# voxel-tracer/ag-pathtracer

Hardware: AMD Instinct MI355X
Metric: Mrays/sec (primary+secondary) at 1080p/64spp (higher is better)
Workload: dtype f32; 1 GPU; BASELINE configs[2]: Sponza-class closed atrium, 258672 tris / 37 primitives / 35 Disney materials, 1920x1080, 64 spp, PathTracer MaxDepth=5, NEE+MIS; triangles=258672, spp=64

## Files before the change

### ag-pathtracer_amd/csrc/agpt_api.hip

```cpp
#include <hip/hip_runtime.h>

#include <algorithm>
#include <cstdlib>
#include <cstring>
#include <memory>
#include <string>
#include <vector>

#include "agpt_adaptive.h"
#include "agpt_denoise.h"
#include "agpt_internal.h"
#include "agpt_kernels.h"
#include "agpt_motion.h"

namespace agpt {

static thread_local std::string g_error;

int fail(int code, const std::string& msg) {
    g_error = msg;
    return code;
}

int interleave_rows(int H, int block, int world, int rank) {
// ... 209 lines not shown
    if (!c || !dst || !src) return fail(AGPT_ERR_INVALID, "agpt_device_download: NULL argument");
    HIP_TRY(hipMemcpyAsync(dst, src, bytes, hipMemcpyDeviceToHost, c->stream));
    HIP_TRY(hipStreamSynchronize(c->stream));
    return AGPT_OK;
}
int agpt_device_upload(agpt_ctx* c, void* dst, const void* src, size_t bytes) {
    if (!c || !dst || !src) return fail(AGPT_ERR_INVALID, "agpt_device_upload: NULL argument");
    HIP_TRY(hipMemcpyAsync(dst, src, bytes, hipMemcpyHostToDevice, c->stream));
    HIP_TRY(hipStreamSynchronize(c->stream));
    return AGPT_OK;
}

#define X(T, name) +sizeof(T)
constexpr size_t AGPT_BYTES_PER_PATH = (0 AGPT_POOL_BUFFERS(X)) + 2 * AGPT_NQUEUES * sizeof(uint32_t);
#undef X
static_assert(AGPT_BYTES_PER_PATH == 240, "11 float4 arrays + 2 hit arrays (16 B) + 2 flag words + 6 queue words");
static size_t candidate_bytes_per_path(int n_prims) { return n_prims > 64 ? 4 + 8 * (size_t)((n_prims + 63) / 64) : 0; }
static int ensure_pool(agpt_ctx* c, size_t paths, int n_prims) {
    int rc;
    paths = std::max(paths, c->pool_paths);
    if (n_prims > 64) {
        if ((rc = c->cand_chunks.ensure(paths))) return rc;
        if ((rc = c->cand_mask.ensure(paths * (size_t)((n_prims + 63) / 64)))) return rc;
    }
#define X(T, name) \
    if ((rc = c->name.ensure(paths))) return rc;
    AGPT_POOL_BUFFERS(X)
#undef X
    for (int i = 0; i < 2; i++)
        for (int j = 0; j < AGPT_NQUEUES; j++)
            if ((rc = c->q[i][j].ensure(paths))) return rc;
// ... 100 lines not shown
            uint32_t* slot = c->host_pinned + (it & 1) * (AGPT_NQUEUES * AGPT_QSTRIDE);
            HIP_TRY(hipMemcpyAsync(slot, q[cur].counts, ((AGPT_NQUEUES - 1) * AGPT_QSTRIDE + 1) * sizeof(uint32_t), hipMemcpyDeviceToHost, main_stream));
            HIP_TRY(hipEventRecord(c->ev[2 + (it & 1)], main_stream));
            if (it > planned) {
                const uint32_t* seen = c->host_pinned + ((it - 1) & 1) * (AGPT_NQUEUES * AGPT_QSTRIDE);
                HIP_TRY(hipEventSynchronize(c->ev[2 + ((it - 1) & 1)]));
                if (seen[0] == 0 && seen[AGPT_QSTRIDE] == 0 && seen[2 * AGPT_QSTRIDE] == 0) break;
            }
            if (it > 4096) return fail(AGPT_ERR_LIMIT, "agpt: path did not terminate");
        }
        const int nxt = cur ^ 1;
        HIP_TRY(hipMemsetAsync(q[nxt].counts, 0, AGPT_NQUEUES * AGPT_QSTRIDE * sizeof(uint32_t), main_stream));
        HIP_TRY(hipMemsetAsync(c->work.p, 0, 4 * AGPT_FRONTIERS * AGPT_QSTRIDE * sizeof(uint32_t), main_stream));
        uint32_t* const heads[4] = {c->work.p, c->work.p + AGPT_FRONTIERS * AGPT_QSTRIDE, c->work.p + 2 * AGPT_FRONTIERS * AGPT_QSTRIDE,
                                    c->work.p + 3 * AGPT_FRONTIERS * AGPT_QSTRIDE};
        const TraceLaunch ext{main_stream, q[cur].ext, &QCOUNT(q[cur], 0), 0, heads[0], pb.ext_o, pb.ext_d, pb.hit, nullptr,
                              count, small_batch, recast, coherent && it == 0};
        const TraceLaunch mis{mis_stream, q[cur].mis, &QCOUNT(q[cur], 1), 0, heads[1], pb.mis_o, pb.mis_d,
                              run.mis_mode ? nullptr : pb.mis_hit, run.mis_mode ? pb.mis_ok : nullptr, count, small_batch, false, false};
        const TraceLaunch shadow{shadow_stream, q[cur].shadow, &QCOUNT(q[cur], 2), 0, heads[2], pb.sh_o, pb.sh_d, nullptr, pb.occluded,
                                 count, small_batch, false, false};
        auto trace_ext = [&]() { launch_trace_timed<0>(c, run.timing, 0, s->dev, ext); };
        auto trace_mis = [&]() {
            if (run.mis_mode) launch_trace_timed<2>(c, run.timing, 1, s->dev, mis);
            else launch_trace_timed<0>(c, run.timing, 1, s->dev, mis);
        };
        auto trace_shadow = [&]() { launch_trace_timed<1>(c, run.timing, 2, s->dev, shadow); };
        if (side) {
            HIP_TRY(hipEventRecord(c->aux_ev[0], main_stream));
            HIP_TRY(hipStreamWaitEvent(mis_stream, c->aux_ev[0], 0));
            HIP_TRY(hipStreamWaitEvent(shadow_stream, c->aux_ev[0], 0));
            trace_mis();
            HIP_TRY(hipEventRecord(c->aux_ev[1], mis_stream));
            trace_shadow();
            HIP_TRY(hipEventRecord(c->aux_ev[2], shadow_stream));
            trace_ext();
            HIP_TRY(hipStreamWaitEvent(main_stream, c->aux_ev[1], 0));
            HIP_TRY(hipStreamWaitEvent(main_stream, c->aux_ev[2], 0));
        } else {
            trace_ext();
            trace_mis();
            trace_shadow();
        }
        agpt::launch_shading(main_stream, run.shade, shade_grid, s->dev, rcn, pb, q[cur], q[nxt], c->counters.p, heads[3]);
        cur = nxt;
        run.iterations++;
        run.launches += 3;
    }
    return AGPT_OK;
}

static void read_counters(const DevCounters& d, agpt_stats* st) {
    st->closest_rays = d.closest_rays;
    st->anyhit_rays = d.anyhit_rays;
    st->interior_visits = d.interior;
    st->root_tests = d.roots;
    st->tri_tests = d.tris;
    st->shaded_vertices = d.shaded;
    st->outliers = d.outliers;
// ... 419 lines not shown
```

### ag-pathtracer_amd/csrc/agpt_internal.h

```cpp
#pragma once

#include <hip/hip_runtime.h>

#include <string>
#include <utility>
#include <vector>

#include "../../include/agpt.h"
#include "agpt_host_scene.hpp"
#include "agpt_update.h"
#include "agpt_wavefront.h"

#ifndef AGPT_FAST_STACK
#define AGPT_FAST_STACK 23
#endif
#ifndef AGPT_FAST_BLOCKS_PER_CU
#define AGPT_FAST_BLOCKS_PER_CU 5
#endif
#define AGPT_REFILL 20
#define AGPT_REFILL_ANY 40

namespace agpt {
int fail(int code, const std::string& msg);
int interleave_rows(int H, int block, int world, int rank);
// ... 42 lines not shown
    }
    int in(const T* host, size_t count) {
        HIP_TRY(alloc(count));
        HIP_TRY(hipMemcpy(p, host, count * sizeof(T), hipMemcpyHostToDevice));
        return AGPT_OK;
    }
    int out(T* host, size_t count, const hipStream_t* st = nullptr) const {
        if (st) HIP_TRY(hipMemcpyAsync(host, p, count * sizeof(T), hipMemcpyDeviceToHost, *st));
        else HIP_TRY(hipMemcpy(host, p, count * sizeof(T), hipMemcpyDeviceToHost));
        return AGPT_OK;
    }
};

#define AGPT_POOL_BUFFERS(X)                                                                                                  \
    X(float4, ext_o) X(float4, ext_d) X(float4, sh_o) X(float4, sh_d) X(float4, mis_o) X(float4, mis_d) X(float4, beta4)      \
    X(float4, L4) X(float4, fac4) X(float4, c1) X(float4, c2) X(DevHit, hit) X(DevHit, mis_hit) X(uint32_t, occluded)          \
    X(uint32_t, mis_ok)

struct agpt_ctx {
    int device = 0;
    hipStream_t stream = nullptr;
    int num_cus = 256;
    hipEvent_t ev[4] = {nullptr, nullptr, nullptr, nullptr};
    hipStream_t aux_stream[2] = {nullptr, nullptr};
    hipEvent_t aux_ev[3] = {nullptr, nullptr, nullptr};
    int multi_stream = 0;
    size_t pool_paths = 0;
#define X(T, name) DevBuf<T> name;
    AGPT_POOL_BUFFERS(X)
#undef X
    DevBuf<uint32_t> q[2][AGPT_NQUEUES];
// ... 111 lines not shown
```

### ag-pathtracer_amd/csrc/agpt_kernels.h

```cpp
#pragma once

#include <type_traits>

#include "agpt_shade.h"
#include "agpt_trace.h"

#include "agpt_wavefront.h"

template <bool ANY, bool COUNT, int DEPTH>
__global__ void __launch_bounds__(AGPT_BLOCK)
k_trace(DevScene sc, const uint32_t* __restrict__ queue, const uint32_t* __restrict__ count_ptr, uint32_t count_imm,
        uint32_t* __restrict__ work_head, const float4* __restrict__ ray_o, const float4* __restrict__ ray_d,
        DevHit* __restrict__ hits, uint32_t* __restrict__ occluded, DevCounters* __restrict__ counters) {
    __shared__ uint32_t s_stack[DEPTH * AGPT_BLOCK];
    uint32_t* stack = s_stack + threadIdx.x;
    const int lane = threadIdx.x & 63;
    const uint32_t count = count_ptr ? *count_ptr : count_imm;
    TraceCounters cnt;
    cnt.interior = 0;
    cnt.tris = 0;
    cnt.roots = 0;
    cnt.last_mesh = 0;
    for (;;) {
        uint32_t base = 0;
// ... 307 lines not shown
    for (;;) {
        TCK(const unsigned long long tk_r0 = TCK_NOW();)
        pin_state();
        any_slow = uni(any_slow);
        if constexpr (MODE == 0 && !LIST) {
            if (__ballot(cur == CUR_RECAST) != 0 && cur == CUR_RECAST) {
                const v3 p = r.O + rayt * r.D;
                const v3 nO = p + AGPT_EPSILON * r.D;
                const v3 nD = normalize(r.D);
                const TraceRay nr = make_trace_ray(nO, nD, coords_ok);
                if (nr.fast) {
                    const float kind = ray_d[pid].w;
                    if (kind == 2.f) {
                        const int al = sc.prims[hid & 0x7FFFFFFFu].arealight;
                        const v3 Le = al >= 0 ? V3(sc.lights[al].L[0], sc.lights[al].L[1], sc.lights[al].L[2]) : V3s(0.f);
                        const float4 b4 = path_beta4[pid];
                        float4 l4 = path_L4[pid];
                        const v3 L = V3(l4.x, l4.y, l4.z) + V3(b4.x, b4.y, b4.z) * Le;
                        l4.x = L.x; l4.y = L.y; l4.z = L.z;
                        path_L4[pid] = l4;
                    }
                    float4 no4, nd4;
                    no4.x = nO.x; no4.y = nO.y; no4.z = nO.z; no4.w = AGPT_FLT_MAX;
                    nd4.x = nD.x; nd4.y = nD.y; nd4.z = nD.z; nd4.w = kind;
                    ray_o[pid] = no4;
                    ray_d[pid] = nd4;
                    atomicAdd(&counters->closest_rays, 1ull);
                    r = nr;
                    rayt = AGPT_FLT_MAX;
                    hid = AGPT_HIT_MISS;
                    hb1 = 0.f;
                    hb2 = 0.f;
                    sp = 0;
// ... 497 lines not shown
    float py = y + rng_float(rng);
    float s = px / rc.W, t = py / rc.H;
    v3 O, D;
    camera_sample_ray(sc.cam, s, t, rng, O, D);
    start_path(pb, q, i, total, O, D, AGPT_FLT_MAX, rng, rc.max_depth);
}

__global__ void __launch_bounds__(AGPT_BLOCK)
k_generate_li(const agpt_ray* __restrict__ rays, const uint32_t* __restrict__ rng_states, uint32_t n, PathBuffers pb, Queues q, int max_depth) {
    const uint32_t i = blockIdx.x * blockDim.x + threadIdx.x;
    if (i >= n) return;
    const agpt_ray r = rays[i];
    const v3 d = normalize(V3(r.d[0], r.d[1], r.d[2]));
    start_path(pb, q, i, n, V3(r.o[0], r.o[1], r.o[2]), d, r.tmax, rng_states[i], max_depth);
}

__global__ void k_resolve(const float4* __restrict__ accum, int n, int samples, uint32_t* __restrict__ out) {
    int i = blockIdx.x * blockDim.x + threadIdx.x;
    if (i >= n) return;
    out[i] = resolve_word(accum[i], (float)samples);
}
```

### ag-pathtracer_amd/csrc/agpt_shade_kernels.h

```cpp
#pragma once

#include "agpt_shade.h"
#include "agpt_trace.h"
#include "agpt_wavefront.h"

#define AGPT_SHADE_LEVEL_LIST(X) X(0, ) X(1, _textured) X(2, _mapped) X(3, _sampled) X(4, _normal)
#ifndef AGPT_SHADE_LEVEL
#define AGPT_SHADE_LEVEL 0
#endif
#if AGPT_SHADE_FAST
#define AGPT_SHADE_FAST_SUFFIX _fast
#else
#define AGPT_SHADE_FAST_SUFFIX
#endif
#define AGPT_SHADE_NTH_0(s0, ...) s0
#define AGPT_SHADE_NTH_1(s0, s1, ...) s1
#define AGPT_SHADE_NTH_2(s0, s1, s2, ...) s2
#define AGPT_SHADE_NTH_3(s0, s1, s2, s3, ...) s3
#define AGPT_SHADE_NTH_4(s0, s1, s2, s3, s4, ...) s4
#define AGPT_SHADE_SUFFIX_ARG(level, suffix) suffix,
#define AGPT_SHADE_CAT_(a, b, c) a##b##c
#define AGPT_SHADE_CAT(a, b, c) AGPT_SHADE_CAT_(a, b, c)
#define AGPT_SHADE_NTH(n, list) AGPT_SHADE_CAT(AGPT_SHADE_NTH_, n, )(list)
#define AGPT_SHADE_KNAME(n) AGPT_SHADE_CAT(n, AGPT_SHADE_NTH(AGPT_SHADE_LEVEL, AGPT_SHADE_LEVEL_LIST(AGPT_SHADE_SUFFIX_ARG)), AGPT_SHADE_FAST_SUFFIX)

#define SB_EXT 1u
#define SB_MIS 2u
#define SB_SHADOW 4u
#define SB_SHADED 32u
#define SB_MIS_ANSWERED 64u
#define SB_RAY_ANSWERED 128u

__device__ __forceinline__ v3 pending_light_sample(const DevScene& sc, const RenderConsts& rc, const PathBuffers& pb, uint32_t pid,
                                                   uint32_t flags, uint32_t was_occluded, uint32_t was_mis_ok, float4 c1_4, float4 c2_4,
                                                   float4 f4) {
    v3 Ld = V3s(0.f);
    if (flags & PF_PEND_C1) {
        if (!was_occluded) {
            Ld = Ld + V3(c1_4.x, c1_4.y, c1_4.z);
        }
    }
    if (flags & PF_PEND_C2) {
        uint32_t light = __float_as_uint(f4.w);
        bool add;
        if (rc.mis_mode) {
            add = was_mis_ok != 0;
        } else if (uint32_t hid = pb.mis_hit[pid].id; hid != AGPT_HIT_MISS) {
            int hp = (hid & AGPT_HIT_SPHERE) ? (int)(hid & 0x7FFFFFFFu)
                                             : (int)__float_as_uint(sc.tri_shade[4 * (size_t)hid + 3].w);
            add = sc.prims[hp].arealight == (int)light;
        } else {
            add = sc.lights[light].type != AGPT_LIGHT_AREA;
        }
        if (add) Ld = Ld + V3(c2_4.x, c2_4.y, c2_4.z);
    }
    return Ld;
}

#ifdef AGPT_SHADE_CLOCK
#define SCK_PARAMS , unsigned long long* sck_acc, unsigned long long& sck_last
#define SCK_ARGS , sck_acc, sck_last
#define SCK(k) do { asm volatile("s_waitcnt vmcnt(0) lgkmcnt(0)" ::: "memory"); const unsigned long long sck_now = __builtin_amdgcn_s_memtime(); \
                    sck_acc[k] += sck_now - sck_last; sck_last = sck_now; } while (0)
#else
#define SCK_PARAMS
#define SCK_ARGS
#define SCK(k)
#endif
template <bool ENV, bool TEXTURED = (AGPT_SHADE_LEVEL >= 1), bool MAPPED = (AGPT_SHADE_LEVEL >= 2), bool SAMPLED = (AGPT_SHADE_LEVEL >= 3),
          bool NORMAL = (AGPT_SHADE_LEVEL == 4)>
__device__ __forceinline__ uint32_t shade_path(const DevScene& sc, const RenderConsts& rc, const PathBuffers& pb, uint32_t pid,
                                               const int32_t* normal_table SCK_PARAMS) {
    uint32_t bits = 0;
    float4 b4 = pb.beta4[pid];
    float4 l4 = pb.L4[pid];
    const float4 f4 = pb.fac4[pid];
    const uint32_t was_occluded = pb.occluded[pid];
    const uint32_t was_mis_ok = pb.mis_ok[pid];
    const float4 c1_4 = pb.c1[pid], c2_4 = pb.c2[pid];
    const DevHit h = pb.hit[pid];
    const float4 o4 = pb.ext_o[pid], d4 = pb.ext_d[pid];
    v3 beta = V3(b4.x, b4.y, b4.z);
    v3 L = V3(l4.x, l4.y, l4.z);
    uint32_t flags = __float_as_uint(b4.w);
    uint32_t rng = __float_as_uint(l4.w);

    SCK(0);
    asm volatile("" : "+v"(pid));
    if (flags & PF_PENDING) {
        const v3 Ld = pending_light_sample(sc, rc, pb, pid, flags, was_occluded, was_mis_ok, c1_4, c2_4, f4);
        float lightPdf = sh_rcp(sc.n_lights);
        L = L + beta * sh_div3(Ld, lightPdf);
        if (!(flags & PF_DEAD)) beta = beta * V3(f4.x, f4.y, f4.z);
        flags &= ~(PF_PENDING | PF_PEND_C1 | PF_PEND_C2);
    }

    SCK(1);
    if (!(flags & PF_DEAD)) {
        uint32_t bounces = flags & PF_BOUNCE_MASK;
        v3 O = V3(o4.x, o4.y, o4.z), D = V3(d4.x, d4.y, d4.z);
        const bool found = h.id != AGPT_HIT_MISS;
        Surface s;
        float4 uv01 = {0.f, 0.f, 0.f, 0.f}, uv2 = {0.f, 0.f, 0.f, 0.f};
        if (found) {
            if (h.id & AGPT_HIT_SPHERE)
                surface_from_sphere(sc, (int)(h.id & 0x7FFFFFFFu), O, D, h.t, s);
            else {
                if constexpr (TEXTURED) {
// ... 220 lines not shown
                if (eval) {
                    const bool reflect = dot(wi, bsdf.ng) * woDotNg > 0;
                    const LobeEval e = bsdf_eval_lobes_inl(m, lmask, wo_l, wi_l, skip_lobe, pdf, reflect, wc);
                    if (it == 0)
                        pdf = matching > 0 ? sh_div(e.pdf, matching) : 0.f;
                    else if (matching > 1)
                        pdf = sh_div(e.pdf, matching);
                    if (reflect) f = e.f;
                }
                if (it == 0) {
                    scatteringPdf = pdf;
                    f = f * absdot(wi, s.ns);
                    if (!isblack(f)) {
                        float weight = power_heuristic(1, nee_lightPdf, 1, scatteringPdf);
                        v3 c1 = sh_div3(f * nee_Li * weight, nee_lightPdf);
                        float4 c4;
                        c4.x = c1.x; c4.y = c1.y; c4.z = c1.z; c4.w = 0.f;
                        pb.c1[pid] = c4;
                        flags |= PF_PEND_C1;
                        bits |= SB_SHADOW;
                    }
                } else if (it == 1) {
                    const DevLight& light = sc.lights[numLight];
                    f = f * absdot(wi, s.ns);
                    if (!isblack(f) && pdf > 0) {
                        float lp;
                        if (light.type == AGPT_LIGHT_UNIFORM_INFINITE)
                            lp = dot(s.n, wi) > 0 ? AGPT_INV2PI : 0.f;
                        else if (ENV && light.type == AGPT_LIGHT_INFINITE_AREA)
                            lp = env_pdf_li(&sc.envs[light.env], wi);
                        else
                            lp = sphere_pdf(sc.prims[light.shape], s.p);
                        if (lp != 0) {
// ... 3 lines not shown
                            v3 c2 = isblack(Li2) ? V3s(0.f) : sh_div3(f * Li2 * weight, pdf);
                            v3 mO = s.p + AGPT_EPSILON * wi;
                            v3 mD = normalize(wi);
                            bool reach = true;
                            if (rc.answer_rays && light.type == AGPT_LIGHT_AREA) {
                                const DevPrim& LS = sc.prims[light.shape];
                                TraceRay qr;
                                qr.O = mO;
                                qr.D = mD;
                                float ts;
                                reach = sphere_test_c(V3(LS.cx, LS.cy, LS.cz), LS.r2, qr, AGPT_FLT_MAX, ts);
                            }
                            if (!reach) {
                                bits |= SB_MIS_ANSWERED;
                            } else {
                            float4 c4, mo4, md4;
                            c4.x = c2.x; c4.y = c2.y; c4.z = c2.z; c4.w = 0.f;
                            mo4.x = mO.x; mo4.y = mO.y; mo4.z = mO.z;
                            mo4.w = rc.mis_mode ? __uint_as_float(light.type == AGPT_LIGHT_AREA ? (uint32_t)light.shape : 0xFFFFFFFFu)
                                                : AGPT_FLT_MAX;
                            md4.x = mD.x; md4.y = mD.y; md4.z = mD.z; md4.w = __uint_as_float((uint32_t)numLight);
                            pb.c2[pid] = c4;
                            pb.mis_o[pid] = mo4;
                            pb.mis_d[pid] = md4;
                            flags |= PF_PEND_C2;
                            bits |= SB_MIS;
                            }
                        }
                    }
                } else if (isblack(f) || pdf == 0) {
                    flags |= PF_DEAD;
                } else {
                    fac = sh_div3(f * absdot(wi, s.ns), pdf);
                    if (!(flags & PF_PENDING)) beta = beta * fac;
                    flags = (flags & ~PF_SPECULAR) | (sampledSpecular ? PF_SPECULAR : 0u);
                    flags = (flags & ~PF_BOUNCE_MASK) | ((bounces + 1) & PF_BOUNCE_MASK);
                    if (rc.answer_rays && (int)(bounces + 1) >= rc.max_depth && !sampledSpecular) {
// ... 1 lines not shown
                        bits |= SB_RAY_ANSWERED;
                    } else {
                        v3 nO = s.p + AGPT_EPSILON * wi;
                        v3 nD = normalize(wi);
                        float4 no4, nd4;
                        no4.x = nO.x; no4.y = nO.y; no4.z = nO.z; no4.w = AGPT_FLT_MAX;
                        nd4.x = nD.x; nd4.y = nD.y; nd4.z = nD.z;
                        nd4.w = (!sampledSpecular && (int)(bounces + 1) < rc.max_depth) ? 1.f : 0.f;
                        pb.ext_o[pid] = no4;
                        pb.ext_d[pid] = nd4;
                        bits |= SB_EXT;
                    }
                }
            }
            SCK(5);
            if (flags & PF_PENDING) {
                float4 f4;
                f4.x = fac.x; f4.y = fac.y; f4.z = fac.z; f4.w = __uint_as_float((uint32_t)numLight);
                pb.fac4[pid] = f4;
            }
        }
    }
    b4.x = beta.x; b4.y = beta.y; b4.z = beta.z; b4.w = __uint_as_float(flags);
    pb.beta4[pid] = b4;
    l4.x = L.x; l4.y = L.y; l4.z = L.z; l4.w = __uint_as_float(rng);
    pb.L4[pid] = l4;
    SCK(6);
    return bits;
}

#ifndef SHADE_GRAB
#define SHADE_GRAB 2
#endif
#ifndef SHADE_U
#define SHADE_U 4
#endif

#ifndef AGPT_SHADE_WAVES
#define AGPT_SHADE_WAVES 3
#endif
#define AGPT_SHADE_LDS_PRIMS 256
#define AGPT_SHADE_LDS_MATERIALS 128
#define AGPT_SHADE_LDS_LIGHTS 64
template <bool LDS_TABLES, bool ENV>
__global__ void __launch_bounds__(AGPT_BLOCK, AGPT_SHADE_WAVES)
AGPT_SHADE_KNAME(k_shade)(DevScene sc_in, RenderConsts rc, PathBuffers pb, Queues qin, Queues qout, DevCounters* __restrict__ counters,
        uint32_t* __restrict__ tile_heads) {
    __shared__ DevPrim s_tab_prims[LDS_TABLES ? AGPT_SHADE_LDS_PRIMS : 1];
    __shared__ DevMaterial s_tab_materials[LDS_TABLES ? AGPT_SHADE_LDS_MATERIALS : 1];
    __shared__ DevLight s_tab_lights[LDS_TABLES ? AGPT_SHADE_LDS_LIGHTS : 1];
#if AGPT_SHADE_LEVEL
    constexpr int n_tab_halves = AGPT_SHADE_LEVEL >= 2 ? 2 : 1;
    __shared__ int32_t s_tab_material_texture[LDS_TABLES ? n_tab_halves * AGPT_SHADE_LDS_MATERIALS : 1];
#endif
    if (blockIdx.x * (AGPT_BLOCK / 64) * 64u * SHADE_U >= QCOUNT(qin, 0) && blockIdx.x > 0) return;
    DevScene sc = sc_in;
    if (LDS_TABLES) {
        auto copy_words = [&](void* dst, const void* src, int n_bytes) {
            uint32_t* d = (uint32_t*)dst;
            const uint32_t* g = (const uint32_t*)src;
            for (int i = threadIdx.x; i < n_bytes / 4; i += AGPT_BLOCK) d[i] = g[i];
        };
// ... 56 lines not shown
                }
            }
        }
        return false;
    };
    for (uint32_t t = 0; next_tile(t);) {
        uint32_t total[AGPT_NQUEUES] = {0, 0, 0};
#pragma unroll 1
        for (int u = 0; u < SHADE_U; ++u) {
#ifdef AGPT_SHADE_CLOCK
            { const unsigned long long n0 = __builtin_amdgcn_s_memtime(); sck_acc[7] += n0 - sck_last; sck_last = n0; }
#endif
            const uint32_t qi = t * wtile + (uint32_t)u * 64u + (uint32_t)lane;
            uint32_t pid = 0, bits = 0;
            if (qi < n_active) {
                pid = qin.ext[qi];
                bits = shade_path<ENV>(sc, rc, pb, pid, AGPT_SHADE_LEVEL == 4 ? sc_in.material_texture : nullptr SCK_ARGS);
            }
            s_pid[u][tid] = pid;
            s_bits[u][tid] = bits;
            shaded += (bits & SB_SHADED) ? 1u : 0u;
            mis_answered += ((bits & SB_MIS_ANSWERED) ? 1u : 0u) + ((bits & SB_RAY_ANSWERED) ? 1u : 0u);
            for (int q = 0; q < AGPT_NQUEUES; ++q) total[q] += (uint32_t)__popcll(__ballot((bits >> q) & 1u));
        }
        uint32_t my_total = total[0];
        for (int q = 1; q < AGPT_NQUEUES; ++q) my_total = lane == q ? total[q] : my_total;
        uint32_t base = 0;
        if (lane < AGPT_NQUEUES && my_total) base = atomicAdd(&QCOUNT(qout, lane), my_total);
        uint32_t run[AGPT_NQUEUES];
        for (int q = 0; q < AGPT_NQUEUES; ++q) run[q] = (uint32_t)__shfl((int)base, q);
        for (int u = 0; u < SHADE_U; ++u) {
            const uint32_t bits = s_bits[u][tid];
// ... 13 lines not shown
    if (lane == 0) {
        for (int k = 0; k < 8; ++k) atomicAdd(&counters->dbg[56 + k], sck_acc[k]);
        atomicAdd(&counters->dbg[55], __builtin_amdgcn_s_memtime() - sck_begin);
    }
#endif
    for (int off = 32; off > 0; off >>= 1) {
        shaded += __shfl_down(shaded, off);
        mis_answered += __shfl_down(mis_answered, off);
    }
    if (lane == 0 && shaded) atomicAdd(&counters->shaded, (unsigned long long)shaded);
    if (lane == 0 && mis_answered) {
        atomicAdd(&counters->closest_rays, (unsigned long long)mis_answered);
        atomicAdd(&counters->answered, (unsigned long long)mis_answered);
    }
}

__device__ __forceinline__ v3 finished_radiance(const DevScene& sc, const RenderConsts& rc, const PathBuffers& pb, uint32_t pid, float4 b4,
                                                float4 l4) {
    const v3 L = V3(l4.x, l4.y, l4.z);
    const uint32_t flags = __float_as_uint(b4.w);
    if (!(flags & PF_PENDING)) return L;
    const uint32_t was_occluded = pb.occluded[pid], was_mis_ok = pb.mis_ok[pid];
    const float4 c1_4 = pb.c1[pid], c2_4 = pb.c2[pid];
    float4 f4 = {0.f, 0.f, 0.f, 0.f};
    if (!rc.mis_mode) f4 = pb.fac4[pid];
    const v3 Ld = pending_light_sample(sc, rc, pb, pid, flags, was_occluded, was_mis_ok, c1_4, c2_4, f4);
    const float lightPdf = sh_rcp(sc.n_lights);
    return L + V3(b4.x, b4.y, b4.z) * sh_div3(Ld, lightPdf);
}

#if !AGPT_SHADE_LEVEL
__global__ void __launch_bounds__(AGPT_BLOCK)
AGPT_SHADE_KNAME(k_accumulate)(DevScene sc, RenderConsts rc, PathBuffers pb, float4* __restrict__ accum, DevCounters* __restrict__ counters) {
    __shared__ float4 s_clr[AGPT_BLOCK];
    const uint32_t G = sample_group(rc.S), per_block = AGPT_BLOCK / G;
    const uint32_t tid = threadIdx.x;
    const uint32_t p0 = blockIdx.x * per_block;
    const uint32_t pf = p0 + tid / G;
    const bool owner = tid < per_block && p0 + tid < rc.NP;
    float4 a = {0.f, 0.f, 0.f, 0.f};
    size_t ai = 0;
// ... 46 lines not shown
    const uint32_t i = blockIdx.x * blockDim.x + threadIdx.x;
    if (i >= n) return;
    float4 b4 = pb.beta4[i];
    const uint32_t flags = __float_as_uint(b4.w);
    if (!(flags & PF_PENDING)) return;
    float4 l4 = pb.L4[i];
    const v3 L = finished_radiance(sc, rc, pb, i, b4, l4);
    l4.x = L.x; l4.y = L.y; l4.z = L.z;
    pb.L4[i] = l4;
    b4.w = __uint_as_float(flags & ~(PF_PENDING | PF_PEND_C1 | PF_PEND_C2));
    pb.beta4[i] = b4;
}
#endif

namespace agpt {
using ShadeLaunch = void(hipStream_t stream, int grid, bool lds_tables, bool env, const DevScene& sc, const RenderConsts& rc,
                         const PathBuffers& pb, const Queues& qin, const Queues& qout, DevCounters* counters, uint32_t* tile_heads);
using AccumulateLaunch = void(hipStream_t stream, const DevScene& sc, const RenderConsts& rc, const PathBuffers& pb, float4* accum,
                               DevCounters* counters);
using FinishPathsLaunch = void(hipStream_t stream, const DevScene& sc, const RenderConsts& rc, const PathBuffers& pb, uint32_t n);
#define X(level, suffix) ShadeLaunch launch_shade##suffix, launch_shade##suffix##_fast;
AGPT_SHADE_LEVEL_LIST(X)
#undef X
AccumulateLaunch finish_accumulate, finish_accumulate_fast;
FinishPathsLaunch finish_paths, finish_paths_fast;
using ExportLiLaunch = void(hipStream_t stream, const DevScene& sc, const RenderConsts& rc, const PathBuffers& pb, uint32_t n, float* radiance3,
                            uint32_t* rng_out);
ExportLiLaunch finish_export_li, finish_export_li_fast;

void AGPT_SHADE_KNAME(launch_shade)(hipStream_t stream, int grid, bool lds_tables, bool env, const DevScene& sc, const RenderConsts& rc,
                                    const PathBuffers& pb, const Queues& qin, const Queues& qout, DevCounters* counters,
                                    uint32_t* tile_heads) {
    const dim3 g(grid), b(AGPT_BLOCK);
    if (lds_tables && env)
        hipLaunchKernelGGL((AGPT_SHADE_KNAME(k_shade)<true, true>), g, b, 0, stream, sc, rc, pb, qin, qout, counters, tile_heads);
    else if (lds_tables)
        hipLaunchKernelGGL((AGPT_SHADE_KNAME(k_shade)<true, false>), g, b, 0, stream, sc, rc, pb, qin, qout, counters, tile_heads);
    else if (env)
        hipLaunchKernelGGL((AGPT_SHADE_KNAME(k_shade)<false, true>), g, b, 0, stream, sc, rc, pb, qin, qout, counters, tile_heads);
    else
        hipLaunchKernelGGL((AGPT_SHADE_KNAME(k_shade)<false, false>), g, b, 0, stream, sc, rc, pb, qin, qout, counters, tile_heads);
}
#if !AGPT_SHADE_LEVEL
void AGPT_SHADE_KNAME(finish_accumulate)(hipStream_t stream, const DevScene& sc, const RenderConsts& rc, const PathBuffers& pb, float4* accum,
                                         DevCounters* counters) {
    hipLaunchKernelGGL(AGPT_SHADE_KNAME(k_accumulate), agpt_blocks((uint64_t)rc.NP * sample_group(rc.S))   , dim3(AGPT_BLOCK), 0, stream, sc, rc, pb, accum, counters);
}
void AGPT_SHADE_KNAME(finish_paths)(hipStream_t stream, const DevScene& sc, const RenderConsts& rc, const PathBuffers& pb, uint32_t n) {
    hipLaunchKernelGGL(AGPT_SHADE_KNAME(k_resolve_pending), agpt_blocks(n), dim3(AGPT_BLOCK), 0, stream, sc, rc, pb, n);
// ... 8 lines not shown
```

### ag-pathtracer_amd/csrc/agpt_shade_kernels.hip

```cpp
#define AGPT_SHADE_LEVEL 0
#define AGPT_SHADE_FAST 0
#include <hip/hip_runtime.h>

#include "agpt_shade_kernels.h"

namespace agpt {

bool shade_tables_fit_lds(int n_prims, int n_materials, int n_lights) {
    return n_prims <= AGPT_SHADE_LDS_PRIMS && n_materials <= AGPT_SHADE_LDS_MATERIALS && n_lights <= AGPT_SHADE_LDS_LIGHTS;
}

void launch_shading(hipStream_t stream, const ShadeVariant& v, int shade_grid, const DevScene& sc, const RenderConsts& rc,
                    const PathBuffers& pb, const Queues& qin, const Queues& qout, DevCounters* counters, uint32_t* tile_heads) {
#define X(level, suffix) {launch_shade##suffix, launch_shade##suffix##_fast},
    static ShadeLaunch* const table[SHADE_LEVELS][2] = {AGPT_SHADE_LEVEL_LIST(X)};
#undef X
    table[v.level][v.fast](stream, shade_grid, v.lds_tables, v.env, sc, rc, pb, qin, qout, counters, tile_heads);
}

void launch_accumulate(hipStream_t stream, bool fast, const DevScene& sc, const RenderConsts& rc, const PathBuffers& pb, float4* accum,
                       DevCounters* counters) {
    (fast ? finish_accumulate_fast : finish_accumulate)(stream, sc, rc, pb, accum, counters);
}
void launch_export_li(hipStream_t stream, bool fast, const DevScene& sc, const RenderConsts& rc, const PathBuffers& pb, uint32_t n,
                      float* radiance3, uint32_t* rng_out) {
    (fast ? finish_export_li_fast : finish_export_li)(stream, sc, rc, pb, n, radiance3, rng_out);
}
void launch_finish_paths(hipStream_t stream, bool fast, const DevScene& sc, const RenderConsts& rc, const PathBuffers& pb, uint32_t n) {
    (fast ? finish_paths_fast : finish_paths)(stream, sc, rc, pb, n);
}

}
// ... 1 lines not shown
```

### ag-pathtracer_amd/csrc/agpt_wavefront.h

```cpp
#pragma once

#include "agpt_math.h"
#include "agpt_scene.h"

#define AGPT_BLOCK 256
#define AGPT_CHUNK 64

#define PF_BOUNCE_MASK 0xFFu
#define PF_SPECULAR 0x100u
#define PF_DEAD 0x200u
#define PF_PEND_C1 0x400u
#define PF_PEND_C2 0x800u
#define PF_PENDING 0x1000u

struct PathBuffers {
    float4 *ext_o, *ext_d;
    float4 *sh_o, *sh_d;
    float4 *mis_o, *mis_d;
    DevHit *hit, *mis_hit;
    uint32_t* occluded;
    uint32_t* mis_ok;
    float4* beta4;
    float4* L4;
    float4* fac4;
    float4 *c1, *c2;
};

#define AGPT_QSTRIDE 32
#ifndef AGPT_FRONTIERS
#define AGPT_FRONTIERS 8u
#endif
struct Queues {
    uint32_t *ext, *mis, *shadow;
    uint32_t* counts;
};
#define AGPT_NQUEUES 3
#define QCOUNT(q, i) ((q).counts[(i) * AGPT_QSTRIDE])

struct RenderConsts {
    int32_t W, H, x0, y0, w, h;
// ... 49 lines not shown
    v3 rd = V3s(0.f);
    if (c.lens_radius > 0.f) {
        for (;;) {
            float a = -1.f + (1.f - -1.f) * rng_float(rng);
            float b = -1.f + (1.f - -1.f) * rng_float(rng);
            v3 pd = V3(a, b, 0);
            if (sqrlen(pd) >= 1) continue;
            rd = c.lens_radius * pd;
            break;
        }
    }
    camera_ray(c, s, t, rd.x, rd.y, O, D);
}
__device__ __forceinline__ void start_path(const PathBuffers& pb, const Queues& q, uint32_t i, uint32_t total, v3 O, v3 D, float tmax,
                                           uint32_t rng, int32_t max_depth) {
    float4 o4, d4, b4, l4;
    o4.x = O.x; o4.y = O.y; o4.z = O.z; o4.w = tmax;
    d4.x = D.x; d4.y = D.y; d4.z = D.z;
    d4.w = max_depth > 0 ? 2.f : 0.f;
    b4.x = 1.f; b4.y = 1.f; b4.z = 1.f; b4.w = __uint_as_float(0u);
    l4.x = 0.f; l4.y = 0.f; l4.z = 0.f; l4.w = __uint_as_float(rng);
    pb.ext_o[i] = o4;
    pb.ext_d[i] = d4;
    pb.beta4[i] = b4;
    pb.L4[i] = l4;
    q.ext[i] = i;
    if (i == 0) {
        QCOUNT(q, 0) = total;
        QCOUNT(q, 1) = 0;
        QCOUNT(q, 2) = 0;
    }
}
struct FilmSample { v3 clr; uint32_t bad; };
__device__ __forceinline__ FilmSample film_sample(v3 clr, uint32_t bad) {
    if (isnan(clr.x) || isnan(clr.y) || isnan(clr.z) || isinf(luminance(clr))) {
        clr = V3s(0.f);
        bad++;
    }
    return FilmSample{clr, bad};
}
__device__ __forceinline__ uint32_t resolve_word(const float4& a, float n) {
    float e = 1 / 2.2f;
    float r = powf(a.x / n, e), g = powf(a.y / n, e), b = powf(a.z / n, e);
    int ri = (int)(256 * tclampf(r, 0.0f, 0.999f));
    int gi = (int)(256 * tclampf(g, 0.0f, 0.999f));
    int bi = (int)(256 * tclampf(b, 0.0f, 0.999f));
// ... 37 lines not shown
    base = __shfl(base, leader);
    if (pred) {
        uint32_t off = (uint32_t)__popcll(mask & ((1ull << lane) - 1ull));
        q[base + off] = value;
    }
}


namespace agpt {
bool shade_tables_fit_lds(int n_prims, int n_materials, int n_lights);
enum ShadeLevel { SHADE_PLAIN = 0, SHADE_TEXTURED = 1, SHADE_MAPPED = 2, SHADE_SAMPLED = 3, SHADE_NORMAL = 4, SHADE_LEVELS = 5 };
struct ShadeVariant {
    ShadeLevel level;
    bool fast, lds_tables, env;
};
void launch_shading(hipStream_t stream, const ShadeVariant& v, int shade_grid, const DevScene& sc, const RenderConsts& rc,
                    const PathBuffers& pb, const Queues& qin, const Queues& qout, DevCounters* counters, uint32_t* tile_heads);
void launch_accumulate(hipStream_t stream, bool fast, const DevScene& sc, const RenderConsts& rc, const PathBuffers& pb, float4* accum,
                       DevCounters* counters);
void launch_export_li(hipStream_t stream, bool fast, const DevScene& sc, const RenderConsts& rc, const PathBuffers& pb, uint32_t n,
                      float* radiance3, uint32_t* rng_out);
void launch_finish_paths(hipStream_t stream, bool fast, const DevScene& sc, const RenderConsts& rc, const PathBuffers& pb, uint32_t n);
void launch_kat_bsdf_eval_fast(hipStream_t stream, const DevScene& sc, int material, int n, const float* wo3, const float* wi3, float* f3o,
                               float* pdfo);
void launch_kat_bsdf_sample_fast(hipStream_t stream, const DevScene& sc, int material, int n, const float* wo3, const float* u2, float* wi3o,
                                 float* f3o, float* pdfo, int32_t* speco);
void launch_kat_env_light_fast(hipStream_t stream, const DevScene& sc, int light, int n_dirs, const float* d3, float* le3o, float* pdf_li_o,
                               int n_draws, const float* u, float* wi3o, float* pdfo, float* sle3o, int32_t* oko);
}
```

Measured before the change: 4520 Mrays/s.

## Shrink per-path light state to float3 and specialize first-bounce shading

The per-path NEE factor and the two pending-contribution buffers change from float4 to float3, and the light index is now read from mis_d.w. This cuts per-path pool bytes and the global load/store traffic in shading. A FIRST template twin of the LDS-table shade kernel assumes beta is one and no pending light state, using the queue index directly as the path id. Paths without LDS tables get beta and queue entries from a new kernel instead of start_path. This adds kernel variants and depends on the first-hit emission path in the trace kernel staying correct now that beta is taken as one.

```diff
diff --git a/ag-pathtracer_amd/csrc/agpt_api.hip b/ag-pathtracer_amd/csrc/agpt_api.hip
--- a/ag-pathtracer_amd/csrc/agpt_api.hip
+++ b/ag-pathtracer_amd/csrc/agpt_api.hip
@@ -247,7 +247,7 @@
 #define X(T, name) +sizeof(T)
 constexpr size_t AGPT_BYTES_PER_PATH = (0 AGPT_POOL_BUFFERS(X)) + 2 * AGPT_NQUEUES * sizeof(uint32_t);
 #undef X
-static_assert(AGPT_BYTES_PER_PATH == 240, "11 float4 arrays + 2 hit arrays (16 B) + 2 flag words + 6 queue words");
+static_assert(AGPT_BYTES_PER_PATH == 228, "8 float4 arrays + 3 float3 arrays (12 B) + 2 hit arrays (16 B) + 2 flag words + 6 queue words");
 static size_t candidate_bytes_per_path(int n_prims) { return n_prims > 64 ? 4 + 8 * (size_t)((n_prims + 63) / 64) : 0; }
 static int ensure_pool(agpt_ctx* c, size_t paths, int n_prims) {
     int rc;
@@ -378,7 +378,10 @@
         HIP_TRY(hipMemsetAsync(c->work.p, 0, 4 * AGPT_FRONTIERS * AGPT_QSTRIDE * sizeof(uint32_t), main_stream));
         uint32_t* const heads[4] = {c->work.p, c->work.p + AGPT_FRONTIERS * AGPT_QSTRIDE, c->work.p + 2 * AGPT_FRONTIERS * AGPT_QSTRIDE,
                                     c->work.p + 3 * AGPT_FRONTIERS * AGPT_QSTRIDE};
-        const TraceLaunch ext{main_stream, q[cur].ext, &QCOUNT(q[cur], 0), 0, heads[0], pb.ext_o, pb.ext_d, pb.hit, nullptr,
+        const bool first = it == 0;
+        if (first && !run.shade.lds_tables)
+            hipLaunchKernelGGL(k_first_vertex_state, dim3(c->num_cus * 8), dim3(AGPT_BLOCK), 0, main_stream, pb, q[cur]);
+        const TraceLaunch ext{main_stream, first ? nullptr : q[cur].ext, &QCOUNT(q[cur], 0), 0, heads[0], pb.ext_o, pb.ext_d, pb.hit, nullptr,
                               count, small_batch, recast, coherent && it == 0};
         const TraceLaunch mis{mis_stream, q[cur].mis, &QCOUNT(q[cur], 1), 0, heads[1], pb.mis_o, pb.mis_d,
                               run.mis_mode ? nullptr : pb.mis_hit, run.mis_mode ? pb.mis_ok : nullptr, count, small_batch, false, false};
@@ -406,7 +409,7 @@
             trace_mis();
             trace_shadow();
         }
-        agpt::launch_shading(main_stream, run.shade, shade_grid, s->dev, rcn, pb, q[cur], q[nxt], c->counters.p, heads[3]);
+        agpt::launch_shading(main_stream, run.shade, first, shade_grid, s->dev, rcn, pb, q[cur], q[nxt], c->counters.p, heads[3]);
         cur = nxt;
         run.iterations++;
         run.launches += 3;
diff --git a/ag-pathtracer_amd/csrc/agpt_internal.h b/ag-pathtracer_amd/csrc/agpt_internal.h
--- a/ag-pathtracer_amd/csrc/agpt_internal.h
+++ b/ag-pathtracer_amd/csrc/agpt_internal.h
@@ -80,7 +80,7 @@
 
 #define AGPT_POOL_BUFFERS(X)                                                                                                  \
     X(float4, ext_o) X(float4, ext_d) X(float4, sh_o) X(float4, sh_d) X(float4, mis_o) X(float4, mis_d) X(float4, beta4)      \
-    X(float4, L4) X(float4, fac4) X(float4, c1) X(float4, c2) X(DevHit, hit) X(DevHit, mis_hit) X(uint32_t, occluded)          \
+    X(float4, L4) X(float3, fac3) X(float3, c1) X(float3, c2) X(DevHit, hit) X(DevHit, mis_hit) X(uint32_t, occluded)          \
     X(uint32_t, mis_ok)
 
 struct agpt_ctx {
diff --git a/ag-pathtracer_amd/csrc/agpt_kernels.h b/ag-pathtracer_amd/csrc/agpt_kernels.h
--- a/ag-pathtracer_amd/csrc/agpt_kernels.h
+++ b/ag-pathtracer_amd/csrc/agpt_kernels.h
@@ -345,9 +345,8 @@
                     if (kind == 2.f) {
                         const int al = sc.prims[hid & 0x7FFFFFFFu].arealight;
                         const v3 Le = al >= 0 ? V3(sc.lights[al].L[0], sc.lights[al].L[1], sc.lights[al].L[2]) : V3s(0.f);
-                        const float4 b4 = path_beta4[pid];
                         float4 l4 = path_L4[pid];
-                        const v3 L = V3(l4.x, l4.y, l4.z) + V3(b4.x, b4.y, b4.z) * Le;
+                        const v3 L = V3(l4.x, l4.y, l4.z) + V3s(1.f) * Le;
                         l4.x = L.x; l4.y = L.y; l4.z = L.z;
                         path_L4[pid] = l4;
                     }
@@ -875,6 +874,11 @@
     const v3 d = normalize(V3(r.d[0], r.d[1], r.d[2]));
     start_path(pb, q, i, n, V3(r.o[0], r.o[1], r.o[2]), d, r.tmax, rng_states[i], max_depth);
 }
+__global__ void __launch_bounds__(AGPT_BLOCK)
+k_first_vertex_state(PathBuffers pb, Queues q) {
+    const uint32_t n = QCOUNT(q, 0);
+    for (uint32_t i = blockIdx.x * blockDim.x + threadIdx.x; i < n; i += gridDim.x * blockDim.x) first_vertex_state(pb, q, i);
+}
 
 __global__ void k_resolve(const float4* __restrict__ accum, int n, int samples, uint32_t* __restrict__ out) {
     int i = blockIdx.x * blockDim.x + threadIdx.x;
diff --git a/ag-pathtracer_amd/csrc/agpt_shade_kernels.h b/ag-pathtracer_amd/csrc/agpt_shade_kernels.h
--- a/ag-pathtracer_amd/csrc/agpt_shade_kernels.h
+++ b/ag-pathtracer_amd/csrc/agpt_shade_kernels.h
@@ -31,28 +31,27 @@
 #define SB_MIS_ANSWERED 64u
 #define SB_RAY_ANSWERED 128u
 
+__device__ __forceinline__ uint32_t pending_light(const PathBuffers& pb, uint32_t pid) { return __float_as_uint(pb.mis_d[pid].w); }
 __device__ __forceinline__ v3 pending_light_sample(const DevScene& sc, const RenderConsts& rc, const PathBuffers& pb, uint32_t pid,
-                                                   uint32_t flags, uint32_t was_occluded, uint32_t was_mis_ok, float4 c1_4, float4 c2_4,
-                                                   float4 f4) {
+                                                   uint32_t flags, uint32_t was_occluded, uint32_t was_mis_ok, float3 c1_3, float3 c2_3) {
     v3 Ld = V3s(0.f);
     if (flags & PF_PEND_C1) {
         if (!was_occluded) {
-            Ld = Ld + V3(c1_4.x, c1_4.y, c1_4.z);
+            Ld = Ld + V3(c1_3.x, c1_3.y, c1_3.z);
         }
     }
     if (flags & PF_PEND_C2) {
-        uint32_t light = __float_as_uint(f4.w);
         bool add;
         if (rc.mis_mode) {
             add = was_mis_ok != 0;
-        } else if (uint32_t hid = pb.mis_hit[pid].id; hid != AGPT_HIT_MISS) {
+        } else if (uint32_t hid = pb.mis_hit[pid].id, light = pending_light(pb, pid); hid != AGPT_HIT_MISS) {
             int hp = (hid & AGPT_HIT_SPHERE) ? (int)(hid & 0x7FFFFFFFu)
                                              : (int)__float_as_uint(sc.tri_shade[4 * (size_t)hid + 3].w);
             add = sc.prims[hp].arealight == (int)light;
         } else {
             add = sc.lights[light].type != AGPT_LIGHT_AREA;
         }
-        if (add) Ld = Ld + V3(c2_4.x, c2_4.y, c2_4.z);
+        if (add) Ld = Ld + V3(c2_3.x, c2_3.y, c2_3.z);
     }
     return Ld;
 }
@@ -67,17 +66,22 @@
 #define SCK_ARGS
 #define SCK(k)
 #endif
-template <bool ENV, bool TEXTURED = (AGPT_SHADE_LEVEL >= 1), bool MAPPED = (AGPT_SHADE_LEVEL >= 2), bool SAMPLED = (AGPT_SHADE_LEVEL >= 3),
+template <bool ENV, bool FIRST, bool TEXTURED = (AGPT_SHADE_LEVEL >= 1), bool MAPPED = (AGPT_SHADE_LEVEL >= 2), bool SAMPLED = (AGPT_SHADE_LEVEL >= 3),
           bool NORMAL = (AGPT_SHADE_LEVEL == 4)>
 __device__ __forceinline__ uint32_t shade_path(const DevScene& sc, const RenderConsts& rc, const PathBuffers& pb, uint32_t pid,
                                                const int32_t* normal_table SCK_PARAMS) {
     uint32_t bits = 0;
-    float4 b4 = pb.beta4[pid];
+    float4 b4 = {1.f, 1.f, 1.f, __uint_as_float(0u)};
+    float3 f3 = {0.f, 0.f, 0.f}, c1_3 = f3, c2_3 = f3;
+    uint32_t was_occluded = 0, was_mis_ok = 0;
+    if constexpr (!FIRST) b4 = pb.beta4[pid];
     float4 l4 = pb.L4[pid];
-    const float4 f4 = pb.fac4[pid];
-    const uint32_t was_occluded = pb.occluded[pid];
-    const uint32_t was_mis_ok = pb.mis_ok[pid];
-    const float4 c1_4 = pb.c1[pid], c2_4 = pb.c2[pid];
+    if constexpr (!FIRST) {
+        f3 = pb.fac3[pid];
+        was_occluded = pb.occluded[pid];
+        was_mis_ok = pb.mis_ok[pid];
+        c1_3 = pb.c1[pid], c2_3 = pb.c2[pid];
+    }
     const DevHit h = pb.hit[pid];
     const float4 o4 = pb.ext_o[pid], d4 = pb.ext_d[pid];
     v3 beta = V3(b4.x, b4.y, b4.z);
@@ -87,11 +91,11 @@
 
     SCK(0);
     asm volatile("" : "+v"(pid));
-    if (flags & PF_PENDING) {
-        const v3 Ld = pending_light_sample(sc, rc, pb, pid, flags, was_occluded, was_mis_ok, c1_4, c2_4, f4);
+    if (!FIRST && (flags & PF_PENDING)) {
+        const v3 Ld = pending_light_sample(sc, rc, pb, pid, flags, was_occluded, was_mis_ok, c1_3, c2_3);
         float lightPdf = sh_rcp(sc.n_lights);
         L = L + beta * sh_div3(Ld, lightPdf);
-        if (!(flags & PF_DEAD)) beta = beta * V3(f4.x, f4.y, f4.z);
+        if (!(flags & PF_DEAD)) beta = beta * V3(f3.x, f3.y, f3.z);
         flags &= ~(PF_PENDING | PF_PEND_C1 | PF_PEND_C2);
     }
 
@@ -342,9 +346,9 @@
                     if (!isblack(f)) {
                         float weight = power_heuristic(1, nee_lightPdf, 1, scatteringPdf);
                         v3 c1 = sh_div3(f * nee_Li * weight, nee_lightPdf);
-                        float4 c4;
-                        c4.x = c1.x; c4.y = c1.y; c4.z = c1.z; c4.w = 0.f;
-                        pb.c1[pid] = c4;
+                        float3 c3;
+                        c3.x = c1.x; c3.y = c1.y; c3.z = c1.z;
+                        pb.c1[pid] = c3;
                         flags |= PF_PEND_C1;
                         bits |= SB_SHADOW;
                     }
@@ -378,13 +382,14 @@
                             if (!reach) {
                                 bits |= SB_MIS_ANSWERED;
                             } else {
-                            float4 c4, mo4, md4;
-                            c4.x = c2.x; c4.y = c2.y; c4.z = c2.z; c4.w = 0.f;
+                            float3 c3;
+                            float4 mo4, md4;
+                            c3.x = c2.x; c3.y = c2.y; c3.z = c2.z;
                             mo4.x = mO.x; mo4.y = mO.y; mo4.z = mO.z;
                             mo4.w = rc.mis_mode ? __uint_as_float(light.type == AGPT_LIGHT_AREA ? (uint32_t)light.shape : 0xFFFFFFFFu)
                                                 : AGPT_FLT_MAX;
                             md4.x = mD.x; md4.y = mD.y; md4.z = mD.z; md4.w = __uint_as_float((uint32_t)numLight);
-                            pb.c2[pid] = c4;
+                            pb.c2[pid] = c3;
                             pb.mis_o[pid] = mo4;
                             pb.mis_d[pid] = md4;
                             flags |= PF_PEND_C2;
@@ -416,10 +421,10 @@
                 }
             }
             SCK(5);
-            if (flags & PF_PENDING) {
-                float4 f4;
-                f4.x = fac.x; f4.y = fac.y; f4.z = fac.z; f4.w = __uint_as_float((uint32_t)numLight);
-                pb.fac4[pid] = f4;
+            if ((flags & PF_PENDING) && !(flags & PF_DEAD)) {
+                float3 fc;
+                fc.x = fac.x; fc.y = fac.y; fc.z = fac.z;
+                pb.fac3[pid] = fc;
             }
         }
     }
@@ -444,10 +449,10 @@
 #define AGPT_SHADE_LDS_PRIMS 256
 #define AGPT_SHADE_LDS_MATERIALS 128
 #define AGPT_SHADE_LDS_LIGHTS 64
-template <bool LDS_TABLES, bool ENV>
-__global__ void __launch_bounds__(AGPT_BLOCK, AGPT_SHADE_WAVES)
-AGPT_SHADE_KNAME(k_shade)(DevScene sc_in, RenderConsts rc, PathBuffers pb, Queues qin, Queues qout, DevCounters* __restrict__ counters,
-        uint32_t* __restrict__ tile_heads) {
+template <bool LDS_TABLES, bool ENV, bool FIRST>
+__device__ __forceinline__ void shade_tiles(const DevScene& sc_in, const RenderConsts& rc, const PathBuffers& pb, const Queues& qin,
+                                            const Queues& qout, DevCounters* __restrict__ counters, uint32_t* __restrict__ tile_heads) {
+    static_assert(LDS_TABLES || !FIRST, "only the LDS-table forms have a FIRST twin");
     __shared__ DevPrim s_tab_prims[LDS_TABLES ? AGPT_SHADE_LDS_PRIMS : 1];
     __shared__ DevMaterial s_tab_materials[LDS_TABLES ? AGPT_SHADE_LDS_MATERIALS : 1];
     __shared__ DevLight s_tab_lights[LDS_TABLES ? AGPT_SHADE_LDS_LIGHTS : 1];
@@ -534,8 +539,8 @@
             const uint32_t qi = t * wtile + (uint32_t)u * 64u + (uint32_t)lane;
             uint32_t pid = 0, bits = 0;
             if (qi < n_active) {
-                pid = qin.ext[qi];
-                bits = shade_path<ENV>(sc, rc, pb, pid, AGPT_SHADE_LEVEL == 4 ? sc_in.material_texture : nullptr SCK_ARGS);
+                pid = FIRST ? qi : qin.ext[qi];
+                bits = shade_path<ENV, FIRST>(sc, rc, pb, pid, AGPT_SHADE_LEVEL == 4 ? sc_in.material_texture : nullptr SCK_ARGS);
             }
             s_pid[u][tid] = pid;
             s_bits[u][tid] = bits;
@@ -579,6 +584,18 @@
         atomicAdd(&counters->answered, (unsigned long long)mis_answered);
     }
 }
+template <bool LDS_TABLES, bool ENV>
+__global__ void __launch_bounds__(AGPT_BLOCK, AGPT_SHADE_WAVES)
+AGPT_SHADE_KNAME(k_shade)(DevScene sc_in, RenderConsts rc, PathBuffers pb, Queues qin, Queues qout, DevCounters* __restrict__ counters,
+        uint32_t* __restrict__ tile_heads) {
+    shade_tiles<LDS_TABLES, ENV, false>(sc_in, rc, pb, qin, qout, counters, tile_heads);
+}
+template <bool ENV>
+__global__ void __launch_bounds__(AGPT_BLOCK, AGPT_SHADE_WAVES)
+AGPT_SHADE_KNAME(k_shade_first)(DevScene sc_in, RenderConsts rc, PathBuffers pb, Queues qin, Queues qout, DevCounters* __restrict__ counters,
+        uint32_t* __restrict__ tile_heads) {
+    shade_tiles<true, ENV, true>(sc_in, rc, pb, qin, qout, counters, tile_heads);
+}
 
 __device__ __forceinline__ v3 finished_radiance(const DevScene& sc, const RenderConsts& rc, const PathBuffers& pb, uint32_t pid, float4 b4,
                                                 float4 l4) {
@@ -586,10 +603,8 @@
     const uint32_t flags = __float_as_uint(b4.w);
     if (!(flags & PF_PENDING)) return L;
     const uint32_t was_occluded = pb.occluded[pid], was_mis_ok = pb.mis_ok[pid];
-    const float4 c1_4 = pb.c1[pid], c2_4 = pb.c2[pid];
-    float4 f4 = {0.f, 0.f, 0.f, 0.f};
-    if (!rc.mis_mode) f4 = pb.fac4[pid];
-    const v3 Ld = pending_light_sample(sc, rc, pb, pid, flags, was_occluded, was_mis_ok, c1_4, c2_4, f4);
+    const float3 c1_3 = pb.c1[pid], c2_3 = pb.c2[pid];
+    const v3 Ld = pending_light_sample(sc, rc, pb, pid, flags, was_occluded, was_mis_ok, c1_3, c2_3);
     const float lightPdf = sh_rcp(sc.n_lights);
     return L + V3(b4.x, b4.y, b4.z) * sh_div3(Ld, lightPdf);
 }
@@ -666,7 +681,7 @@
 #endif
 
 namespace agpt {
-using ShadeLaunch = void(hipStream_t stream, int grid, bool lds_tables, bool env, const DevScene& sc, const RenderConsts& rc,
+using ShadeLaunch = void(hipStream_t stream, int grid, bool lds_tables, bool env, bool first, const DevScene& sc, const RenderConsts& rc,
                          const PathBuffers& pb, const Queues& qin, const Queues& qout, DevCounters* counters, uint32_t* tile_heads);
 using AccumulateLaunch = void(hipStream_t stream, const DevScene& sc, const RenderConsts& rc, const PathBuffers& pb, float4* accum,
                                DevCounters* counters);
@@ -680,11 +695,15 @@
                             uint32_t* rng_out);
 ExportLiLaunch finish_export_li, finish_export_li_fast;
 
-void AGPT_SHADE_KNAME(launch_shade)(hipStream_t stream, int grid, bool lds_tables, bool env, const DevScene& sc, const RenderConsts& rc,
-                                    const PathBuffers& pb, const Queues& qin, const Queues& qout, DevCounters* counters,
-                                    uint32_t* tile_heads) {
+void AGPT_SHADE_KNAME(launch_shade)(hipStream_t stream, int grid, bool lds_tables, bool env, bool first, const DevScene& sc,
+                                    const RenderConsts& rc, const PathBuffers& pb, const Queues& qin, const Queues& qout,
+                                    DevCounters* counters, uint32_t* tile_heads) {
     const dim3 g(grid), b(AGPT_BLOCK);
-    if (lds_tables && env)
+    if (lds_tables && first && env)
+        hipLaunchKernelGGL((AGPT_SHADE_KNAME(k_shade_first)<true>), g, b, 0, stream, sc, rc, pb, qin, qout, counters, tile_heads);
+    else if (lds_tables && first)
+        hipLaunchKernelGGL((AGPT_SHADE_KNAME(k_shade_first)<false>), g, b, 0, stream, sc, rc, pb, qin, qout, counters, tile_heads);
+    else if (lds_tables && env)
         hipLaunchKernelGGL((AGPT_SHADE_KNAME(k_shade)<true, true>), g, b, 0, stream, sc, rc, pb, qin, qout, counters, tile_heads);
     else if (lds_tables)
         hipLaunchKernelGGL((AGPT_SHADE_KNAME(k_shade)<true, false>), g, b, 0, stream, sc, rc, pb, qin, qout, counters, tile_heads);
diff --git a/ag-pathtracer_amd/csrc/agpt_shade_kernels.hip b/ag-pathtracer_amd/csrc/agpt_shade_kernels.hip
--- a/ag-pathtracer_amd/csrc/agpt_shade_kernels.hip
+++ b/ag-pathtracer_amd/csrc/agpt_shade_kernels.hip
@@ -10,12 +10,12 @@
     return n_prims <= AGPT_SHADE_LDS_PRIMS && n_materials <= AGPT_SHADE_LDS_MATERIALS && n_lights <= AGPT_SHADE_LDS_LIGHTS;
 }
 
-void launch_shading(hipStream_t stream, const ShadeVariant& v, int shade_grid, const DevScene& sc, const RenderConsts& rc,
+void launch_shading(hipStream_t stream, const ShadeVariant& v, bool first, int shade_grid, const DevScene& sc, const RenderConsts& rc,
                     const PathBuffers& pb, const Queues& qin, const Queues& qout, DevCounters* counters, uint32_t* tile_heads) {
 #define X(level, suffix) {launch_shade##suffix, launch_shade##suffix##_fast},
     static ShadeLaunch* const table[SHADE_LEVELS][2] = {AGPT_SHADE_LEVEL_LIST(X)};
 #undef X
-    table[v.level][v.fast](stream, shade_grid, v.lds_tables, v.env, sc, rc, pb, qin, qout, counters, tile_heads);
+    table[v.level][v.fast](stream, shade_grid, v.lds_tables, v.env, first, sc, rc, pb, qin, qout, counters, tile_heads);
 }
 
 void launch_accumulate(hipStream_t stream, bool fast, const DevScene& sc, const RenderConsts& rc, const PathBuffers& pb, float4* accum,
diff --git a/ag-pathtracer_amd/csrc/agpt_wavefront.h b/ag-pathtracer_amd/csrc/agpt_wavefront.h
--- a/ag-pathtracer_amd/csrc/agpt_wavefront.h
+++ b/ag-pathtracer_amd/csrc/agpt_wavefront.h
@@ -22,8 +22,8 @@
     uint32_t* mis_ok;
     float4* beta4;
     float4* L4;
-    float4* fac4;
-    float4 *c1, *c2;
+    float3* fac3;
+    float3 *c1, *c2;
 };
 
 #define AGPT_QSTRIDE 32
@@ -103,22 +103,25 @@
 }
 __device__ __forceinline__ void start_path(const PathBuffers& pb, const Queues& q, uint32_t i, uint32_t total, v3 O, v3 D, float tmax,
                                            uint32_t rng, int32_t max_depth) {
-    float4 o4, d4, b4, l4;
+    float4 o4, d4, l4;
     o4.x = O.x; o4.y = O.y; o4.z = O.z; o4.w = tmax;
     d4.x = D.x; d4.y = D.y; d4.z = D.z;
     d4.w = max_depth > 0 ? 2.f : 0.f;
-    b4.x = 1.f; b4.y = 1.f; b4.z = 1.f; b4.w = __uint_as_float(0u);
     l4.x = 0.f; l4.y = 0.f; l4.z = 0.f; l4.w = __uint_as_float(rng);
     pb.ext_o[i] = o4;
     pb.ext_d[i] = d4;
-    pb.beta4[i] = b4;
     pb.L4[i] = l4;
-    q.ext[i] = i;
     if (i == 0) {
         QCOUNT(q, 0) = total;
         QCOUNT(q, 1) = 0;
         QCOUNT(q, 2) = 0;
     }
+}
+__device__ __forceinline__ void first_vertex_state(const PathBuffers& pb, const Queues& q, uint32_t i) {
+    float4 b4;
+    b4.x = 1.f; b4.y = 1.f; b4.z = 1.f; b4.w = __uint_as_float(0u);
+    pb.beta4[i] = b4;
+    q.ext[i] = i;
 }
 struct FilmSample { v3 clr; uint32_t bad; };
 __device__ __forceinline__ FilmSample film_sample(v3 clr, uint32_t bad) {
@@ -186,7 +189,7 @@
     ShadeLevel level;
     bool fast, lds_tables, env;
 };
-void launch_shading(hipStream_t stream, const ShadeVariant& v, int shade_grid, const DevScene& sc, const RenderConsts& rc,
+void launch_shading(hipStream_t stream, const ShadeVariant& v, bool first, int shade_grid, const DevScene& sc, const RenderConsts& rc,
                     const PathBuffers& pb, const Queues& qin, const Queues& qout, DevCounters* counters, uint32_t* tile_heads);
 void launch_accumulate(hipStream_t stream, bool fast, const DevScene& sc, const RenderConsts& rc, const PathBuffers& pb, float4* accum,
                        DevCounters* counters);
```

After: 4556 Mrays/s, median of 6. No clear change (+0.8%).
